# yanqinJiang/Animate3D

Hardware: AMD Instinct MI355X
Metric: UNet denoise-steps/sec, 4view×16frame×512² MV-VDM @1/2/4/8 GPU (higher is better)
Workload: dtype bf16; 1 GPU; BASELINE config 2: 4 views x 16 frames x 512^2 px (64x64 latent), CFG-doubled batch V=8 videos, one MVUNetMotionModel.forward per step, SD1.5 MV-VDM UNet 1.53 B params, seeded synthetic weights; parallelism=single GPU

## Files before the change

### animate3d_amd/csrc/gemm_common.h

```cpp
#pragma once
#include "common.h"

struct GemmParams {
  const uint16_t* X; int64_t ldx;
  const uint16_t* W; int64_t ldw;
  const float* bias;
  const uint16_t* rowbias; int64_t rb_div;
  const uint16_t* R; int64_t ldr;
  uint16_t* Y; int64_t ldy;
  int64_t M, N, K;
  float alpha, beta;
  int vec16;
  int out_f32;
  int B, H, Wd, Cin, Ho, Wo, stride, up, He, We;
  int64_t tiles_n, tiles_m;
  int ksplit, nk_item;
  float* ws; int64_t ws_bytes;
  const uint16_t* X2; int64_t ldx2; int64_t K1;
};

constexpr int EPI_LINEAR = 0, EPI_GEGLU = 1;

static inline int a3d_gemm_kernel_of(int flags) { return flags & A3D_GEMM_KERNEL_MASK; }
static inline int a3d_gemm_reserved_cus_of(int flags) { return flags & A3D_GEMM_RESERVED_CUS_MASK; }
// ... 101 lines not shown
      const int o = (i * 4) % BIAS_IMG_STRIDE;
      if ((o < BIAS_IMG_ROWBIAS && !bias) || (o >= BIAS_IMG_ROWBIAS && !rowbias)) bz[i] = 0u;
    }
    asm volatile("s_waitcnt lgkmcnt(0)" ::: "memory");
    tile_barrier();
  }
}

template <int NB> A3D_DEV void read_frags(const char* stage, uint32_t xrd, uint32_t wrd, uint32_t wrd_last, uint32_t ko, u32x4_t (&fx)[2],
                                          u32x4_t (&fw)[NB]) {
  const char* xs = stage + xrd;
  const char* ws = stage + wrd;
  const char* wl = stage + wrd_last;
#pragma unroll
  for (int tm = 0; tm < 2; ++tm) fx[tm] = *reinterpret_cast<const u32x4_t*>(xs + tm * 4096 + ko);
#pragma unroll
  for (int tn = 0; tn < NB - 1; ++tn) fw[tn] = *reinterpret_cast<const u32x4_t*>(ws + tn * 4096 + ko);
  fw[NB - 1] = *reinterpret_cast<const u32x4_t*>(wl + ko);
}

template <int EPI, int NB>
A3D_DEV void epilogue_rounded(const GemmParams& p, f32x16_t (&acc)[NB][2], float* const stg, const float* const bias_lds,
                              const uint16_t* const rowbias_lds, const int64_t m0, const int64_t n0, const int wm, const WaveCols<NB> wc,
                              const int lane) {
  const int wblk = wc.first, wblk_last = wc.last;
  auto pass_cols = [&](int ps) { return (2 * ps + 1 < NB) ? 64 : 32; };
  auto pass_col0 = [&](int ps) { return ((2 * ps + 1 < NB) ? wblk + 2 * ps : wblk_last) * 32; };
  const int l31 = lane & 31, g = lane >> 5;
  constexpr int NP = (NB + 1) / 2;
  constexpr int RS = (EPI == EPI_GEGLU) ? 64 : 128;
// ... 196 lines not shown
#pragma unroll
      for (int e = 0; e < 8; ++e) v[e] = epi_scale(v[e], p.alpha);
      const u32x4_t tr = rres[pi & 1][j];
#pragma unroll
      for (int e = 0; e < 4; ++e) { v[2 * e] = epi_axpy(v[2 * e], p.beta, lo16(tr[e])); v[2 * e + 1] = epi_axpy(v[2 * e + 1], p.beta, hi16(tr[e])); }
      u32x4_t o;
#pragma unroll
      for (int e = 0; e < 4; ++e) o[e] = pack16(v[2 * e], v[2 * e + 1]);
      *reinterpret_cast<u32x4_t*>(p.Y + m * p.ldy + n) = o;
    }
    wave_lds_fence();
  }
}


__attribute__((visibility("hidden"))) int A3D_FN(a3d_launch_gemm_pp)(int conv, int epi, int nb, hipStream_t stream, const GemmParams& p, int cus);
__attribute__((visibility("hidden"))) int A3D_FN(a3d_launch_gemm_ring)(int nb, hipStream_t stream, const GemmParams& p, int cus);
```

### animate3d_amd/csrc/gemm_conv.hip

```cpp
#include "gemm_common.h"

namespace {

constexpr int BM = 128, BN = 128;
template <int BKT> struct TileCfg {
  static constexpr int LROW = BKT + 8;
  static constexpr int TILE_ELEMS = 128 * LROW;
  static constexpr int STAGE_BYTES = 2 * 2 * TILE_ELEMS * 2;
  static constexpr int EPI_BYTES = 4 * 32 * 68 * 4;
  static constexpr int SMEM_BYTES = STAGE_BYTES > EPI_BYTES ? STAGE_BYTES : EPI_BYTES;
  static constexpr int CPR = BKT / 8;
  static constexpr int RPT = 256 / CPR;
  static constexpr int NPASS = 128 / RPT;
};



template <int CONV, int EPI, int BKT, bool RES>
__global__ __launch_bounds__(256, (BKT == 64 ? 2 : 3)) void gemm_kernel(const GemmParams p) {
  using TC = TileCfg<BKT>;
  constexpr int LROW = TC::LROW, TILE_ELEMS = TC::TILE_ELEMS, NPASS = TC::NPASS, RPT = TC::RPT, BK = BKT;
  extern __shared__ __attribute__((aligned(16))) uint16_t smem[];
  const int tid = threadIdx.x;
  const int lane = tid & 63, wid = tid >> 6;
// ... 277 lines not shown
            o[1] = pack16(w[2], w[3]);
            *reinterpret_cast<u32x2_t*>(yy + 4 * hh) = o;
          }
        }
      }
    }
  }
  if (tm == 0 && epf) prefetch_residual(1);
  }
}


constexpr int PBM = 256;
constexpr int NOT_ELIGIBLE = -1000;

inline bool gemm_flags_ok(int flags) {
  return !(flags & ~(A3D_GEMM_RESERVED_CUS_MASK | A3D_GEMM_KERNEL_MASK)) && a3d_gemm_kernel_of(flags) <= A3D_GEMM_RING;
}

inline int device_cus() {
  static int cus_of[64] = {0};
  const int dev = a3d_current_device();
  if (cus_of[dev] == 0) {
    int n = 0;
    if (hipDeviceGetAttribute(&n, hipDeviceAttributeMultiprocessorCount, dev) != hipSuccess) return 0;
    cus_of[dev] = n > 0 ? n : 256;
  }
  return cus_of[dev];
}

constexpr int PERSIST_MIN_FILL = 50;
struct PPPlan { int nb, S, cus; int64_t tiles_m, tiles_n; };
// ... 56 lines not shown
    if (p.N % (64 * nb) != 0) continue;
    const int64_t tiles = (p.M / 128) * (p.N / (64 * nb));
    const int64_t rounds = (tiles + out.cus - 1) / out.cus;
    const int64_t cost = rounds * (128 + 64 * nb);
    if (out.nb == 0 || cost < out.cost) { out.nb = nb; out.cost = cost; }
  }
  return out.nb != 0;
}

template <int CONV, int EPI>
int try_launch_persist(hipStream_t stream, GemmParams& p, int flags) {
  PPPlan pl;
  if (!plan_persist<CONV, EPI>(p, flags, p.ws != nullptr, pl)) return NOT_ELIGIBLE;
  p.tiles_m = pl.tiles_m; p.tiles_n = pl.tiles_n;
  p.ksplit = pl.S; p.nk_item = (int)(p.K / 64) / pl.S;
  return A3D_FN(a3d_launch_gemm_pp)(CONV, EPI, pl.nb, stream, p, pl.cus);
}


template <int CONV, int EPI, int BKT, bool RES>
int launch_res(hipStream_t stream, GemmParams& p, int64_t nblk) {
  using TC = TileCfg<BKT>;
  static uint64_t attr_done = 0;
  if (int rc = a3d_once_per_device(attr_done, [] {
        return (int)hipFuncSetAttribute(reinterpret_cast<const void*>(&gemm_kernel<CONV, EPI, BKT, RES>),
                                        hipFuncAttributeMaxDynamicSharedMemorySize, TC::SMEM_BYTES); })) return rc;
  gemm_kernel<CONV, EPI, BKT, RES><<<dim3((unsigned)nblk), dim3(256), TC::SMEM_BYTES, stream>>>(p);
  return a3d_launch_status();
}

template <int CONV, int EPI, int BKT>
int launch_bk(hipStream_t stream, GemmParams& p, int64_t nblk) {
  if constexpr (EPI == EPI_LINEAR) {
    if (p.R != nullptr) return launch_res<CONV, EPI, BKT, true>(stream, p, nblk);
  }
  return launch_res<CONV, EPI, BKT, false>(stream, p, nblk);
}

template <int CONV, int EPI = EPI_LINEAR>
int launch(hipStream_t stream, GemmParams& p, int flags) {
  if (!gemm_flags_ok(flags)) return A3D_EINVAL;
  if constexpr (CONV == 0 && EPI == EPI_LINEAR) {
    RingPlan rp;
    if (plan_ring(p, flags, rp)) {
      PPPlan pl;
      bool ring = true;
      if (a3d_gemm_kernel_of(flags) != A3D_GEMM_RING && plan_persist<CONV, EPI>(p, flags, p.ws != nullptr, pl)) {
        const int64_t tiles = pl.tiles_m * pl.tiles_n * pl.S;
        const int64_t pp_cost = ((tiles + rp.cus_plan - 1) / rp.cus_plan) * (256 + 64 * pl.nb) * RING_VS_PP_PCT;
        ring = pl.S == 1 && rp.cost * 100 < pp_cost;
      }
      if (ring) {
        p.tiles_m = p.M / 128; p.tiles_n = p.N / (64 * rp.nb);
        return A3D_FN(a3d_launch_gemm_ring)(rp.nb, stream, p, rp.cus);
      }
    }
// ... 4 lines not shown
  }
  p.tiles_m = (p.M + BM - 1) / BM;
  p.tiles_n = (p.N + BN - 1) / BN;
  const int64_t nblk = p.tiles_m * p.tiles_n;
  if (nblk <= 0 || nblk > 0x7fffffffLL) return A3D_EINVAL;
  const bool small = (CONV == 0 && p.K <= 640) || nblk < 768;
  if (small) return launch_bk<CONV, EPI, 32>(stream, p, nblk);
  return launch_bk<CONV, EPI, 64>(stream, p, nblk);
}

template <int CONV>
int64_t splitk_ws_bytes(const GemmParams& p, int flags) {
  PPPlan pl;
  GemmParams q = p;
  q.ws = nullptr; q.ws_bytes = 0;
  if (!gemm_flags_ok(flags)) return 0;
  if (!plan_persist<CONV, EPI_LINEAR>(q, flags, true, pl) || pl.S <= 1) return 0;
  return pl.tiles_m * pl.tiles_n * pl.S * pl.nb * 65536;
}

void attach_workspace(GemmParams& p, void* ws, int64_t ws_bytes) {
  if (ws && ws_bytes > 0 && a3d_aligned(16, ws)) { p.ws = (float*)ws; p.ws_bytes = ws_bytes; }
}

GemmParams dense_params(const void* X, int64_t ldx, const void* W, int64_t ldw, const float* bias, const void* rowbias, int64_t rb_div,
                        const void* R, int64_t ldr, void* Y, int64_t ldy, int64_t M, int64_t N, int64_t K, float alpha, float beta,
                        bool out_f32 = false) {
  GemmParams p{};
  p.X = (const uint16_t*)X; p.ldx = ldx; p.W = (const uint16_t*)W; p.ldw = ldw;
  p.bias = bias; p.rowbias = (const uint16_t*)rowbias; p.rb_div = rowbias ? rb_div : 1;
  p.R = (const uint16_t*)R; p.ldr = ldr; p.Y = (uint16_t*)Y; p.ldy = ldy;
// ... 30 lines not shown
  return gemm_entry(stream, X, ldx, W, ldw, bias, rowbias, rb_div, R, ldr, Y, ldy, M, N, K, alpha, beta, flags, nullptr, 0, nullptr);
}

extern "C" int A3D_FN(a3d_gemm_ws)(a3d_stream_t stream, const void* X, int64_t ldx, const void* W, int64_t ldw,
                                const float* bias, const void* rowbias, int64_t rb_div, const void* R, int64_t ldr,
                                void* Y, int64_t ldy, int64_t M, int64_t N, int64_t K, float alpha, float beta, int flags,
                                void* ws, int64_t ws_bytes, int64_t* ws_needed) {
  return gemm_entry(stream, X, ldx, W, ldw, bias, rowbias, rb_div, R, ldr, Y, ldy, M, N, K, alpha, beta, flags, ws, ws_bytes, ws_needed);
}

extern "C" int A3D_FN(a3d_gemm2)(a3d_stream_t stream, const void* X, int64_t ldx, const void* X2, int64_t ldx2, int64_t K1,
                              const void* W, int64_t ldw, const float* bias, void* Y, int64_t ldy, int64_t M, int64_t N, int64_t K, int flags) {
  GemmParams p = dense_params(X, ldx, W, ldw, bias, nullptr, 1, nullptr, 0, Y, ldy, M, N, K, 1.f, 0.f);
  p.X2 = (const uint16_t*)X2; p.ldx2 = ldx2; p.K1 = K1;
  if (!dense_args_ok(p, 16, 8, 8) || !X2 || K1 <= 0 || K1 >= K || K1 % 64 != 0 || ldx2 % 8 != 0 || !a3d_aligned(16, X2)) return A3D_EINVAL;
  if (!gemm_flags_ok(flags)) return A3D_EINVAL;
  if (ldx2 % 64 != 0 || (uint64_t)ldx2 * 16u >= (1ull << 31)) return A3D_EUNSUPPORTED;
  const int rc = try_launch_persist<0, EPI_LINEAR>((hipStream_t)stream, p, flags);
  return rc == NOT_ELIGIBLE ? A3D_EUNSUPPORTED : rc;
}

extern "C" int A3D_FN(a3d_gemm_f32out)(a3d_stream_t stream, const void* X, int64_t ldx, const void* W, int64_t ldw,
                                    const float* bias, float* Y, int64_t ldy, int64_t M, int64_t N, int64_t K, float alpha) {
  GemmParams p = dense_params(X, ldx, W, ldw, bias, nullptr, 1, nullptr, 0, Y, ldy, M, N, K, alpha, 0.f, true);
  if (!dense_args_ok(p, 16, 8, 4)) return A3D_EINVAL;
  return launch<0>((hipStream_t)stream, p, 0);
}

static int conv_entry(a3d_stream_t stream, const void* X, const void* Wp, const float* bias,
                      const void* rowbias, int64_t rb_div, const void* R, void* Y,
                      int B, int H, int W, int Cin, int Cout, int stride, int up2x, int flags,
// ... 42 lines not shown
```

### animate3d_amd/csrc/gemm_pp.hip

```cpp
#include "gemm_common.h"

namespace {

constexpr int PBM = 256;
template <int NB> struct PPCfg {
  static constexpr int BN = NB * 64;
  static constexpr int XBYTES = PBM * 128;
  static constexpr int WBYTES = BN * 128;
  static constexpr int EPI_BYTES = 8 * 32 * 68 * 4;
  static constexpr int STAGE = (XBYTES + WBYTES) > EPI_BYTES ? (XBYTES + WBYTES) : EPI_BYTES;
  static constexpr int BIAS_OFF = 2 * STAGE;
  static constexpr int SMEM = BIAS_OFF + 2 * BIAS_IMG_STRIDE;
};

constexpr int PP_GM = 8;
A3D_DEV void pp_tile_coords(int64_t t, int64_t tiles_m, int64_t tiles_n, int64_t& tile_m, int64_t& tile_n) {
  const int64_t gsz = PP_GM * tiles_n;
  const int64_t blk = t / gsz;
  const int64_t first = blk * PP_GM;
  const int64_t gm = tiles_m - first < PP_GM ? tiles_m - first : PP_GM;
  const int64_t within = t - blk * gsz;
  tile_n = within / gm;
  tile_m = first + (within - tile_n * gm);
}

template <int CONV, int EPI, int NB, bool RES, bool SPLIT = false, bool TWO = false>
__global__ __launch_bounds__(512, 1) void gemm_pp_kernel(const GemmParams p) {
  static_assert(!TWO || CONV == 0, "the two-source A operand is a dense-GEMM feature");
  using PC = PPCfg<NB>;
  constexpr int PH = 1, NPH = 4;
  constexpr int NP = 4 + NB;
  extern __shared__ __attribute__((aligned(16))) uint16_t smem[];
  char* const smem_b = reinterpret_cast<char*>(smem);
  const int tid = threadIdx.x, lane = tid & 63;
  const int wid = __builtin_amdgcn_readfirstlane(tid >> 6);
  const int wm = wid >> 1, wn = wid & 1;
  const int grp = wid >> 2;
  const int l31 = lane & 31, g = lane >> 5;
  const int lr = lane >> 3, pos = lane & 7;
  const uint32_t lds0 = lds_addr(smem);

  const int S = SPLIT ? p.ksplit : 1;
  const int64_t ntiles = p.tiles_m * p.tiles_n * S;
  const int64_t G = gridDim.x;
  int64_t t = xcd_remap(blockIdx.x, G);
  if (t >= ntiles) return;
// ... 13 lines not shown
  const int64_t cbias = CONV ? ((int64_t)p.Wd + 1) * p.Cin : 0;
  int64_t ld_m0 = 0, ld_n0 = 0;
  int ld_par = 0;
  int ik0 = 0, itap = 0, ikx = 0, iky = 0;
  uint64_t xck = 0;
  uint64_t zpage = 0;
  if constexpr (CONV != 0) {
    zpage = (uint64_t)(uintptr_t)g_zero_page;
    asm volatile("" : "+s"(zpage));
  }
  uint64_t xk = 0, wk = 0, rbk = 0;
  const uint32_t sx8 = (uint32_t)(p.ldx * 16), sw8 = (uint32_t)(p.ldw * 16);
  uint64_t xk2 = 0;
  const uint32_t vx0b = TWO ? (uint32_t)(lr * p.ldx2 * 2 + ((pos ^ (lr >> 1)) << 4)) : 0u;
  const uint32_t sx8b = TWO ? (uint32_t)(p.ldx2 * 16) : 0u;
  auto setup_tile = [&](int64_t tt) {
    int64_t tile_n, tile_m;
    const int64_t tile_id = SPLIT ? (int64_t)((uint32_t)tt / (uint32_t)S) : tt;
    const int64_t kofs = SPLIT ? (CONV ? ((int64_t)(tt - tile_id * S) * nk / 9) * 64 : (int64_t)(tt - tile_id * S) * nk * 64) : 0;
    pp_tile_coords(tile_id, p.tiles_m, p.tiles_n, tile_m, tile_n);
    ld_m0 = tile_m * PBM; ld_n0 = tile_n * PC::BN;
    ik0 = 0; itap = 0; ikx = 0; iky = 0;
    ld_par ^= 1;
    if constexpr (CONV != 0) xck = (uint64_t)(uintptr_t)p.X - (uint64_t)cbias * 2u + (uint64_t)kofs * 2u;
    if constexpr (CONV == 0) xk = (uint64_t)(uintptr_t)(p.X + (ld_m0 + wid * 32) * p.ldx + kofs);
    if constexpr (TWO) xk2 = (uint64_t)(uintptr_t)(p.X2 + (ld_m0 + wid * 32) * p.ldx2);
    wk = (uint64_t)(uintptr_t)(p.W + (ld_n0 + wid * (NB * 8)) * p.ldw + kofs);
    if (EPI == EPI_LINEAR && p.rowbias) rbk = (uint64_t)(uintptr_t)(p.rowbias + (ld_m0 / p.rb_div) * p.N + ld_n0);
    if constexpr (CONV != 0) {
      amask[0] = 0; amask[1] = 0;
#pragma unroll
      for (int i = 0; i < 4; ++i) {
        const int r = (wid * 4 + i) * 8 + lr;
        const int slot = pos ^ ((r >> 1) & 7);
        const uint32_t m = (uint32_t)ld_m0 + (uint32_t)r;
        const uint32_t hw = (uint32_t)(p.Ho * p.Wo);
        const int b = (int)(m / hw);
        const int rem = (int)(m - (uint32_t)b * hw);
        const int oy = (int)((uint32_t)rem / (uint32_t)p.Wo), ox = rem - oy * p.Wo;
        uint32_t mask = 0;
        if constexpr (CONV == 2) {
          const int sy0 = (oy - 1) >> 1, sx0 = (ox - 1) >> 1;
          aoff[i] = (uint32_t)(((((int64_t)b * p.H + sy0) * p.Wd + sx0) * p.Cin + cbias) * 2 + slot * 16);
#pragma unroll
// ... 25 lines not shown
    constexpr int A = decltype(a_c)::value, B = decltype(b_c)::value;
    if constexpr (A >= B) return;
    const uint32_t dst = lds0 + (uint32_t)buf * PC::STAGE;
    if constexpr (A == 0) {
      if (ik0 == 0) {
        const uint32_t bdst = lds0 + (uint32_t)PC::BIAS_OFF + (uint32_t)ld_par * BIAS_IMG_STRIDE;
        if (p.bias) {
          if (wid == 0) glds16_s((uint32_t)lane * 16u, p.bias + ld_n0, bdst);
          if (NB == 5 && wid == 1) { if (lane < 16) glds16_s((uint32_t)lane * 16u, p.bias + ld_n0 + BIAS_IMG_DMA / 4, bdst + (uint32_t)BIAS_IMG_DMA); }
        }
        if (EPI == EPI_LINEAR && p.rowbias && wid == 2) {
          if (lane < PC::BN / 8) glds16_s((uint32_t)lane * 16u, (const void*)(uintptr_t)rbk, bdst + (uint32_t)BIAS_IMG_ROWBIAS);
        }
      }
    }
    if constexpr (CONV != 0) {
      const int ky = iky, kx = ikx;
      const uint32_t rowb = (uint32_t)(p.Wd * p.Cin * 2), colb = (uint32_t)(p.Cin * 2);
      const uint32_t yE = (uint32_t)((ky + 1) >> 1) * rowb, yO = (uint32_t)(ky >> 1) * rowb;
      const uint32_t xE = (uint32_t)((kx + 1) >> 1) * colb, xO = (uint32_t)(kx >> 1) * colb;
#pragma unroll
      for (int i = 0; i < 4; ++i) {
        if (i < A || i >= B) continue;
        const uint32_t d = dst + (uint32_t)(wid * 4 + i) * 1024u;
        const uint32_t mk = amask[i >> 1];
        uint32_t vo = aoff[i];
        if constexpr (CONV == 2) vo += (((mk >> (18 + 2 * (i & 1))) & 1u) ? yE : yO) + (((mk >> (19 + 2 * (i & 1))) & 1u) ? xE : xO);
        const int bit = itap + 9 * (i & 1);
        if ((sok[i >> 1] >> bit) & 1u) {
          glds16_s(vo, (const void*)(uintptr_t)xck, d);
        } else {
// ... 2 lines not shown
        }
      }
    } else {
      const bool sec = TWO && ik0 >= (int)p.K1;
      const uint32_t vxs = sec ? vx0b : vx0, sxs = sec ? sx8b : sx8;
      const uint64_t xks = sec ? xk2 : xk;
#pragma unroll
      for (int i = 0; i < 4; ++i) {
        if (i < A || i >= B) continue;
        const int pc = wid * 4 + i;
        glds16_s(vxs ^ (uint32_t)((i & 1) << 6), (const void*)(uintptr_t)(xks + (uint64_t)(uint32_t)(i * sxs)), dst + (uint32_t)pc * 1024u);
      }
    }
#pragma unroll
    for (int i = 0; i < NB; ++i) {
      if (4 + i < A || 4 + i >= B) continue;
      const int pc = wid * NB + i;
      glds16_s(vw0 ^ (uint32_t)((pc & 1) << 6), (const void*)(uintptr_t)(wk + (uint64_t)(uint32_t)(i * sw8)), dst + (uint32_t)PC::XBYTES + (uint32_t)pc * 1024u);
    }
    if constexpr (B == NP) {
      if constexpr (CONV != 0) {
        const uint64_t cin2 = (uint64_t)(uint32_t)p.Cin * 2u;
        wk += cin2;
        ++itap;
        if (++ikx == 3) { ikx = 0; ++iky; }
        if (itap == 9) {
          itap = 0; iky = 0; wk -= 9u * cin2 - 128u;
          if constexpr (CONV == 1) xck -= (2u * (uint64_t)(uint32_t)p.Wd + 2u) * cin2;
          xck += 128u;
        } else if constexpr (CONV == 1) {
          xck += ikx == 0 ? ((uint64_t)(uint32_t)p.Wd - 2u) * cin2 : cin2;
        }
      } else {
        if (TWO && ik0 >= (int)p.K1) xk2 += 128; else xk += 128;
        wk += 128;
      }
      ik0 += 64;
    }
  };
  auto issue_phase = [&](int buf, auto ph_c, bool late) __attribute__((always_inline)) {
    constexpr int ph = decltype(ph_c)::value;
    using I0 = std::integral_constant<int, 0>;
    using I3 = std::integral_constant<int, 3>;
    using I5 = std::integral_constant<int, 5>;
    using I6 = std::integral_constant<int, 6>;
    using IN = std::integral_constant<int, NP>;
    if (!late) {
      if constexpr (ph == 0) issue_pieces(buf, I0{}, I3{});
      if constexpr (ph == 1) issue_pieces(buf, I3{}, I6{});
      if constexpr (ph == 2) issue_pieces(buf, I6{}, IN{});
    } else {
      if constexpr (ph == 1) issue_pieces(buf, I0{}, I5{});
      if constexpr (ph == 2) issue_pieces(buf, I5{}, IN{});
    }
  };

  f32x16_t acc[NB][2];
  u32x4_t fx[PH][2], fw[PH][NB];
  auto load_frags = [&](int buf, int ks0) __attribute__((always_inline)) {
#pragma unroll
    for (int s = 0; s < PH; ++s) read_frags<NB>(smem_b + buf * PC::STAGE, xrd, wrd, wrd_last, koff0 ^ (uint32_t)((ks0 + s) << 5), fx[s], fw[s]);
  };
  auto mfma_phase = [&]() __attribute__((always_inline)) {
#pragma unroll
    for (int s = 0; s < PH; ++s)
#pragma unroll
      for (int tn = 0; tn < NB; ++tn)
#pragma unroll
        for (int tm = 0; tm < 2; ++tm) acc[tn][tm] = mfma32(fw[s][tn], fx[s][tm], acc[tn][tm]);
  };

  zero_absent_bias_images<512>(smem_b + PC::BIAS_OFF, p.bias, EPI == EPI_LINEAR ? p.rowbias : nullptr, tid);
  setup_tile(t);
  issue_pieces(0, std::integral_constant<int, 0>{}, std::integral_constant<int, NP>{});
  asm volatile("s_waitcnt vmcnt(0)" ::: "memory");
  tile_barrier();
  int buf = 0;
  for (;;) {
    int64_t tile_n, tile_m;
    pp_tile_coords(SPLIT ? (int64_t)((uint32_t)t / (uint32_t)S) : t, p.tiles_m, p.tiles_n, tile_m, tile_n);
    const int64_t m0 = tile_m * PBM, n0 = tile_n * PC::BN;
    const int64_t tnext = t + G;
#pragma unroll
    for (int a = 0; a < NB; ++a)
#pragma unroll
      for (int b = 0; b < 2; ++b)
#pragma unroll
        for (int r = 0; r < 16; ++r) acc[a][b][r] = 0.f;
    const int cur_par = ld_par;
    if (grp) tile_barrier();
    for (int kt = 0; kt < nk; ++kt) {
      const bool last = kt + 1 >= nk;
      const bool more = !last || tnext < ntiles;
      const bool late = kt == 0;
      static_for<NPH>([&](auto ph_c) __attribute__((always_inline)) {
        constexpr int ph = decltype(ph_c)::value;
        load_frags(buf, ph * PH);
        if (more) {
          if constexpr (ph == 0 || ph == 1) {
            if (last && (late ? ph == 1 : ph == 0)) setup_tile(tnext);
          }
          issue_phase(buf ^ 1, ph_c, late);
          if constexpr (ph == NPH - 1) { if (grp) asm volatile("s_waitcnt vmcnt(0)" ::: "memory"); }
        }
        asm volatile("s_waitcnt lgkmcnt(0)" ::: "memory");
        tile_barrier();
        __builtin_amdgcn_s_setprio(1);
        mfma_phase();
        __builtin_amdgcn_s_setprio(0);
        __builtin_amdgcn_sched_barrier(0);
        if constexpr (ph == NPH - 1) { if (more && !grp) asm volatile("s_waitcnt vmcnt(0)" ::: "memory"); }
        tile_barrier();
      });
      buf ^= 1;
    }
    if (!grp) tile_barrier();

    if constexpr (SPLIT) {
      float* const wsi = p.ws + ((t * 8 + wid) * (NB * 8)) * 256 + lane * 4;
#pragma unroll
      for (int tn = 0; tn < NB; ++tn)
#pragma unroll
        for (int tm = 0; tm < 2; ++tm)
#pragma unroll
          for (int q = 0; q < 4; ++q)
            *reinterpret_cast<float4*>(wsi + ((tn * 2 + tm) * 4 + q) * 256) =
                float4{acc[tn][tm][4 * q], acc[tn][tm][4 * q + 1], acc[tn][tm][4 * q + 2], acc[tn][tm][4 * q + 3]};
    } else {
      float* const stg = reinterpret_cast<float*>(smem_b + (buf ^ 1) * PC::STAGE) + wid * (32 * 68);
      const float* const bias_lds = bias_image(smem_b + PC::BIAS_OFF, cur_par);
      const uint16_t* const rowbias_lds = rowbias_image(smem_b + PC::BIAS_OFF, cur_par);
      if constexpr (EPI == EPI_GEGLU || !RES) epilogue_rounded<EPI, NB>(p, acc, stg, bias_lds, rowbias_lds, m0, n0, wm, wc, lane);
      else epilogue_residual<NB>(p, acc, stg, bias_lds, rowbias_lds, m0, n0, wm, wc, lane);
    }
    if (tnext >= ntiles) break;
    t = tnext;
  }
}

template <int NB>
__global__ __launch_bounds__(512) void splitk_reduce_kernel(const GemmParams p) {
  using PC = PPCfg<NB>;
  const int tid = threadIdx.x, lane = tid & 63, wid = tid >> 6;
  const int wm = wid >> 1, wn = wid & 1, l31 = lane & 31, g = lane >> 5;
  const WaveCols<NB> wc(wn);
  const int S = p.ksplit;
  int64_t tile_n, tile_m;
  pp_tile_coords(blockIdx.x, p.tiles_m, p.tiles_n, tile_m, tile_n);
// ... 26 lines not shown
#pragma unroll
        for (int e = 0; e < 4; ++e) v[e] = epi_scale(v[e], p.alpha);
        if (p.R) {
          const u32x2_t tr = *reinterpret_cast<const u32x2_t*>(p.R + m * p.ldr + n);
          v[0] = epi_axpy(v[0], p.beta, lo16(tr[0])); v[1] = epi_axpy(v[1], p.beta, hi16(tr[0]));
          v[2] = epi_axpy(v[2], p.beta, lo16(tr[1])); v[3] = epi_axpy(v[3], p.beta, hi16(tr[1]));
        }
        u32x2_t o;
        o[0] = pack16(v[0], v[1]);
        o[1] = pack16(v[2], v[3]);
        *reinterpret_cast<u32x2_t*>(p.Y + m * p.ldy + n) = o;
      }
    }
}

template <int CONV, int EPI, int NB, bool RES, bool SPLIT = false, bool TWO = false>
int launch_pp(hipStream_t stream, const GemmParams& p, int cus) {
  using PC = PPCfg<NB>;
  static uint64_t attr_done = 0;
  if (int rc = a3d_once_per_device(attr_done, [] {
        return (int)hipFuncSetAttribute(reinterpret_cast<const void*>(&gemm_pp_kernel<CONV, EPI, NB, RES, SPLIT, TWO>),
                                        hipFuncAttributeMaxDynamicSharedMemorySize, PC::SMEM); })) return rc;
  const int64_t ntiles = p.tiles_m * p.tiles_n * (SPLIT ? p.ksplit : 1);
  const unsigned grid = (unsigned)(ntiles < cus ? ntiles : cus);
  gemm_pp_kernel<CONV, EPI, NB, RES, SPLIT, TWO><<<dim3(grid), dim3(512), PC::SMEM, stream>>>(p);
  if (int rc = a3d_launch_status()) return rc;
  if constexpr (SPLIT) {
    splitk_reduce_kernel<NB><<<dim3((unsigned)(p.tiles_m * p.tiles_n), NB), dim3(512), 0, stream>>>(p);
    return a3d_launch_status();
  }
  return 0;
}

template <int CONV>
int launch_pp_conv(int epi, int nb, hipStream_t stream, const GemmParams& p, int cus) {
  if (epi == EPI_GEGLU) {
    if constexpr (CONV == 0) { if (nb == 4) return launch_pp<0, EPI_GEGLU, 4, false>(stream, p, cus); }
    return A3D_EUNSUPPORTED;
  }
  if constexpr (CONV == 0) {
    if (p.X2 != nullptr) {
      if (p.R || p.ksplit > 1) return A3D_EUNSUPPORTED;
      if (nb == 5) return launch_pp<0, EPI_LINEAR, 5, false, false, true>(stream, p, cus);
      if (nb == 4) return launch_pp<0, EPI_LINEAR, 4, false, false, true>(stream, p, cus);
      return A3D_EUNSUPPORTED;
    }
  }
  if (p.ksplit > 1) {
    if (nb == 5) return launch_pp<CONV, EPI_LINEAR, 5, false, true>(stream, p, cus);
    if (nb == 4) return launch_pp<CONV, EPI_LINEAR, 4, false, true>(stream, p, cus);
    return A3D_EUNSUPPORTED;
  }
  if (nb == 5) return p.R ? launch_pp<CONV, EPI_LINEAR, 5, true>(stream, p, cus) : launch_pp<CONV, EPI_LINEAR, 5, false>(stream, p, cus);
  if (nb == 4) return p.R ? launch_pp<CONV, EPI_LINEAR, 4, true>(stream, p, cus) : launch_pp<CONV, EPI_LINEAR, 4, false>(stream, p, cus);
  return A3D_EUNSUPPORTED;
}

}

int A3D_FN(a3d_launch_gemm_pp)(int conv, int epi, int nb, hipStream_t stream, const GemmParams& p, int cus) {
  if (conv == 0) return launch_pp_conv<0>(epi, nb, stream, p, cus);
  if (conv == 1) return launch_pp_conv<1>(epi, nb, stream, p, cus);
  return launch_pp_conv<2>(epi, nb, stream, p, cus);
}
```

### animate3d_amd/hip_ops.py

```python
from __future__ import annotations

import ctypes
import os
from dataclasses import dataclass
from typing import Optional

import torch

_LIB_PATH = os.path.join(os.path.dirname(os.path.abspath(__file__)), "lib", "libanimate3d_hip.so")
_lib = None

c_i64, c_int, c_f32, c_f64, c_vp = ctypes.c_int64, ctypes.c_int, ctypes.c_float, ctypes.c_double, ctypes.c_void_p


class _RowMapC(ctypes.Structure):
    _fields_ = [("gdiv", c_i64), ("ga", c_i64), ("gb", c_i64), ("seg_len", c_i64), ("seg_stride", c_i64), ("ld", c_i64)]


@dataclass(frozen=True)
class RowMap:
    gdiv: int
    ga: int
    gb: int
    seg_len: int
# ... 273 lines not shown
        assert n % 32 == 0
        h, g = w[:n].reshape(n // 32, 32, *w.shape[1:]), w[n:].reshape(n // 32, 32, *w.shape[1:])
        return torch.stack([h, g], dim=1).reshape(w.shape).contiguous()

    def gemm_geglu(self, x, w_il, bias_il, *, tile128: bool = False):
        x, w_il = self._act(x, "geglu.x"), self._act(w_il, "geglu.w")
        M, K = x.shape
        N2 = w_il.shape[0]
        y = self.empty(M, N2 // 2)
        rc = self.lib.a3d_gemm_geglu_bf16(self._stream(), _p(x), x.stride(0), _p(w_il), w_il.stride(0), _p(bias_il), _p(y), y.stride(0), M, N2, K,
                                          self._gemm_flags(tile128))
        _check(rc, f"a3d_gemm_geglu_bf16 M={M} N2={N2} K={K}")
        return y

    def conv3x3(self, x, B: int, H: int, W: int, w, bias, *, stride: int = 1, up2x: bool = False, rowbias=None, rb_div: int = 1, residual=None,
                up_size=None, tile128: bool = False):
        x, w = self._act(x, "conv.x"), self._act(w, "conv.w")
        Cin = x.shape[1]
        Cout = w.shape[0]
        assert x.is_contiguous() and w.is_contiguous() and x.shape[0] == B * H * W and w.shape[1] == 9 * Cin
        He, We = (2 * H, 2 * W) if up2x else (H, W)
        up_code = 1 if up2x else 0
        if up_size is not None:
            if not up2x or up_size[0] not in (2 * H, 2 * H - 1) or up_size[1] not in (2 * W, 2 * W - 1):
                raise ValueError(f"forced upsample size {tuple(up_size)} is not reachable from {(H, W)} (2x or 2x - 1 per axis)")
            He, We = int(up_size[0]), int(up_size[1])
            up_code |= (2 if He == 2 * H - 1 else 0) | (4 if We == 2 * W - 1 else 0)
        Ho, Wo = (He - 1) // stride + 1, (We - 1) // stride + 1
        y = self.empty(B * Ho * Wo, Cout)
        if residual is not None:
            assert residual.is_contiguous() and residual.shape == y.shape
        if rowbias is not None:
            assert rowbias.is_contiguous() and rowbias.shape[1] == Cout
        flags = self._gemm_flags(tile128)
        args = (self._stream(), _p(x), _p(w), _p(bias), _p(rowbias), rb_div, _p(residual), _p(y), B, H, W, Cin, Cout, stride, up_code, flags)
        if self.split_k and not tile128 and B * Ho * Wo <= 32768:
            key = ("conv", B, H, W, Cin, Cout, stride, up_code, rb_div if rowbias is not None else 0, flags)
            need = self._ws_plan.get(key)
            if need is None:
                q = c_i64(0)
                _check(self.lib.a3d_conv3x3_ws_bf16(*args, None, 0, ctypes.byref(q)), f"a3d_conv3x3_ws_bf16 (query) B={B} H={H} W={W} Cin={Cin} Cout={Cout}")
                need = self._ws_plan[key] = int(q.value)
            if need > 0:
                ws = self._workspace(need)
                _check(self.lib.a3d_conv3x3_ws_bf16(*args, _p(ws), need, None), f"a3d_conv3x3_ws_bf16 B={B} H={H} W={W} Cin={Cin} Cout={Cout}")
                return y, Ho, Wo
        rc = self.lib.a3d_conv3x3_bf16(*args)
        _check(rc, f"a3d_conv3x3_bf16 B={B} H={H} W={W} Cin={Cin} Cout={Cout} stride={stride} up={up2x}")
        return y, Ho, Wo
# ... 410 lines not shown
```

### include/animate3d_hip.h

```cpp
#ifndef ANIMATE3D_HIP_H
#define ANIMATE3D_HIP_H

#include <stdint.h>

#ifdef __cplusplus
extern "C" {
#endif

typedef void* a3d_stream_t;

enum {
  A3D_OK = 0,
  A3D_EINVAL = -1,
  A3D_EUNSUPPORTED = -2
};

enum { A3D_F32 = 0, A3D_BF16 = 1, A3D_F16 = 2 };

const char* a3d_version(void);

typedef struct a3d_rowmap {
  int64_t gdiv, ga, gb;
  int64_t seg_len, seg_stride;
  int64_t ld;
} a3d_rowmap;

#define A3D_GEMM_RESERVED_CUS_MASK 0xff
#define A3D_GEMM_KERNEL_MASK 0x300
#define A3D_GEMM_TILE128 0x100
#define A3D_GEMM_RING 0x200
int a3d_gemm_bf16(a3d_stream_t stream, const void* X, int64_t ldx, const void* W, int64_t ldw,
                  const float* bias, const void* rowbias, int64_t rb_div, const void* R, int64_t ldr,
                  void* Y, int64_t ldy, int64_t M, int64_t N, int64_t K, float alpha, float beta, int flags);

int a3d_gemm_ws_bf16(a3d_stream_t stream, const void* X, int64_t ldx, const void* W, int64_t ldw,
                     const float* bias, const void* rowbias, int64_t rb_div, const void* R, int64_t ldr,
                     void* Y, int64_t ldy, int64_t M, int64_t N, int64_t K, float alpha, float beta, int flags,
                     void* ws, int64_t ws_bytes, int64_t* ws_needed);

int a3d_gemm2_bf16(a3d_stream_t stream, const void* X, int64_t ldx, const void* X2, int64_t ldx2, int64_t K1,
                   const void* W, int64_t ldw, const float* bias, void* Y, int64_t ldy, int64_t M, int64_t N, int64_t K, int flags);

int a3d_gemm_f32out_bf16(a3d_stream_t stream, const void* X, int64_t ldx, const void* W, int64_t ldw,
                         const float* bias, float* Y, int64_t ldy, int64_t M, int64_t N, int64_t K, float alpha);

// ... 291 lines not shown
```

Measured before the change: 2.404 denoise-steps/s.

## Stage conv input row windows in LDS once per K-chunk for stride-1 3x3 convs

Adds a window-staged variant of the persistent implicit-GEMM conv kernel. For stride-1 convs with 64- or 32-wide images and 320-column tiles, it loads the needed input rows into an LDS window once per 64-channel chunk and reads all nine taps from it, instead of re-gathering the A tile from global memory for every tap. This cuts global and L2 traffic for the A operand and frees the X staging area, at the cost of complex row-slot double-buffering and epilogue buffers placed in the window region. A per-tap flag keeps the old path available.

```diff
diff --git a/animate3d_amd/csrc/gemm_common.h b/animate3d_amd/csrc/gemm_common.h
--- a/animate3d_amd/csrc/gemm_common.h
+++ b/animate3d_amd/csrc/gemm_common.h
@@ -139,6 +139,17 @@
   const char* wl = stage + wrd_last;
 #pragma unroll
   for (int tm = 0; tm < 2; ++tm) fx[tm] = *reinterpret_cast<const u32x4_t*>(xs + tm * 4096 + ko);
+#pragma unroll
+  for (int tn = 0; tn < NB - 1; ++tn) fw[tn] = *reinterpret_cast<const u32x4_t*>(ws + tn * 4096 + ko);
+  fw[NB - 1] = *reinterpret_cast<const u32x4_t*>(wl + ko);
+}
+
+template <int NB> A3D_DEV void read_frags_w(const char* stage, const char* xs0, const char* xs1, uint32_t wrd, uint32_t wrd_last, uint32_t ko,
+                                            u32x4_t (&fx)[2], u32x4_t (&fw)[NB]) {
+  const char* ws = stage + wrd;
+  const char* wl = stage + wrd_last;
+  fx[0] = *reinterpret_cast<const u32x4_t*>(xs0);
+  fx[1] = *reinterpret_cast<const u32x4_t*>(xs1);
 #pragma unroll
   for (int tn = 0; tn < NB - 1; ++tn) fw[tn] = *reinterpret_cast<const u32x4_t*>(ws + tn * 4096 + ko);
   fw[NB - 1] = *reinterpret_cast<const u32x4_t*>(wl + ko);
@@ -365,5 +376,5 @@
 }
 
 
-__attribute__((visibility("hidden"))) int A3D_FN(a3d_launch_gemm_pp)(int conv, int epi, int nb, hipStream_t stream, const GemmParams& p, int cus);
+__attribute__((visibility("hidden"))) int A3D_FN(a3d_launch_gemm_pp)(int conv, int epi, int nb, bool win, hipStream_t stream, const GemmParams& p, int cus);
 __attribute__((visibility("hidden"))) int A3D_FN(a3d_launch_gemm_ring)(int nb, hipStream_t stream, const GemmParams& p, int cus);
diff --git a/animate3d_amd/csrc/gemm_conv.hip b/animate3d_amd/csrc/gemm_conv.hip
--- a/animate3d_amd/csrc/gemm_conv.hip
+++ b/animate3d_amd/csrc/gemm_conv.hip
@@ -315,8 +315,8 @@
 constexpr int PBM = 256;
 constexpr int NOT_ELIGIBLE = -1000;
 
-inline bool gemm_flags_ok(int flags) {
-  return !(flags & ~(A3D_GEMM_RESERVED_CUS_MASK | A3D_GEMM_KERNEL_MASK)) && a3d_gemm_kernel_of(flags) <= A3D_GEMM_RING;
+inline bool gemm_flags_ok(int flags, bool conv) {
+  return !(flags & ~(A3D_GEMM_RESERVED_CUS_MASK | A3D_GEMM_KERNEL_MASK | (conv ? A3D_CONV_PER_TAP : 0))) && a3d_gemm_kernel_of(flags) <= A3D_GEMM_RING;
 }
 
 inline int device_cus() {
@@ -403,7 +403,9 @@
   if (!plan_persist<CONV, EPI>(p, flags, p.ws != nullptr, pl)) return NOT_ELIGIBLE;
   p.tiles_m = pl.tiles_m; p.tiles_n = pl.tiles_n;
   p.ksplit = pl.S; p.nk_item = (int)(p.K / 64) / pl.S;
-  return A3D_FN(a3d_launch_gemm_pp)(CONV, EPI, pl.nb, stream, p, pl.cus);
+  const bool win = CONV == 1 && p.stride == 1 && !(flags & A3D_CONV_PER_TAP) && pl.nb == 5 && pl.S == 1 && (p.Wd == 64 || p.Wd == 32) &&
+                   ((int64_t)p.H * p.Wd) % PBM == 0;
+  return A3D_FN(a3d_launch_gemm_pp)(CONV, EPI, pl.nb, win, stream, p, pl.cus);
 }
 
 
@@ -428,7 +430,7 @@
 
 template <int CONV, int EPI = EPI_LINEAR>
 int launch(hipStream_t stream, GemmParams& p, int flags) {
-  if (!gemm_flags_ok(flags)) return A3D_EINVAL;
+  if (!gemm_flags_ok(flags, CONV != 0)) return A3D_EINVAL;
   if constexpr (CONV == 0 && EPI == EPI_LINEAR) {
     RingPlan rp;
     if (plan_ring(p, flags, rp)) {
@@ -463,7 +465,7 @@
   PPPlan pl;
   GemmParams q = p;
   q.ws = nullptr; q.ws_bytes = 0;
-  if (!gemm_flags_ok(flags)) return 0;
+  if (!gemm_flags_ok(flags, CONV != 0)) return 0;
   if (!plan_persist<CONV, EPI_LINEAR>(q, flags, true, pl) || pl.S <= 1) return 0;
   return pl.tiles_m * pl.tiles_n * pl.S * pl.nb * 65536;
 }
@@ -524,7 +526,7 @@
   GemmParams p = dense_params(X, ldx, W, ldw, bias, nullptr, 1, nullptr, 0, Y, ldy, M, N, K, 1.f, 0.f);
   p.X2 = (const uint16_t*)X2; p.ldx2 = ldx2; p.K1 = K1;
   if (!dense_args_ok(p, 16, 8, 8) || !X2 || K1 <= 0 || K1 >= K || K1 % 64 != 0 || ldx2 % 8 != 0 || !a3d_aligned(16, X2)) return A3D_EINVAL;
-  if (!gemm_flags_ok(flags)) return A3D_EINVAL;
+  if (!gemm_flags_ok(flags, false)) return A3D_EINVAL;
   if (ldx2 % 64 != 0 || (uint64_t)ldx2 * 16u >= (1ull << 31)) return A3D_EUNSUPPORTED;
   const int rc = try_launch_persist<0, EPI_LINEAR>((hipStream_t)stream, p, flags);
   return rc == NOT_ELIGIBLE ? A3D_EUNSUPPORTED : rc;
diff --git a/animate3d_amd/csrc/gemm_pp.hip b/animate3d_amd/csrc/gemm_pp.hip
--- a/animate3d_amd/csrc/gemm_pp.hip
+++ b/animate3d_amd/csrc/gemm_pp.hip
@@ -3,15 +3,30 @@
 namespace {
 
 constexpr int PBM = 256;
-template <int NB> struct PPCfg {
+template <int NB, bool WIN = false> struct PPCfg {
   static constexpr int BN = NB * 64;
-  static constexpr int XBYTES = PBM * 128;
+  static constexpr int XBYTES = WIN ? 0 : PBM * 128;
   static constexpr int WBYTES = BN * 128;
-  static constexpr int EPI_BYTES = 8 * 32 * 68 * 4;
-  static constexpr int STAGE = (XBYTES + WBYTES) > EPI_BYTES ? (XBYTES + WBYTES) : EPI_BYTES;
-  static constexpr int BIAS_OFF = 2 * STAGE;
+  static constexpr int EPI_WAVE = 32 * 68 * 4;
+  static constexpr int EPI_BYTES = 8 * EPI_WAVE;
+  static constexpr int STAGE = WIN ? WBYTES : ((XBYTES + WBYTES) > EPI_BYTES ? (XBYTES + WBYTES) : EPI_BYTES);
+  static constexpr int WIN_OFF = 2 * STAGE;
+  static constexpr int WIN_BYTES = WIN ? 16 * 34 * 128 : 0;
+  static constexpr int BIAS_OFF = WIN_OFF + WIN_BYTES;
   static constexpr int SMEM = BIAS_OFF + 2 * BIAS_IMG_STRIDE;
+  static_assert(!WIN || (4 * EPI_WAVE <= WBYTES && 4 * EPI_WAVE <= WIN_BYTES / 2), "window-staged conv: the epilogue buffers do not fit");
+  static_assert(SMEM <= 160 * 1024, "LDS plan exceeds the CU's 160 KB");
 };
+
+constexpr uint64_t win_jobs(int a0, int a1, int a2, int a3, int a4, int a5, int a6, int a7, int a8) {
+  const int a[9] = {a0, a1, a2, a3, a4, a5, a6, a7, a8};
+  uint64_t v = 0;
+  for (int i = 0; i < 9; ++i) v |= (uint64_t)(a[i] & 15) << (4 * i);
+  return v;
+}
+constexpr uint64_t WIN_JOBS_64 = win_jobs(4, 5, 2, 0, 3, 15, 1, 15, 15);
+constexpr uint64_t WIN_JOBS_32E = win_jobs(8, 2, 4, 0, 6, 15, 15, 15, 15);
+constexpr uint64_t WIN_JOBS_32O = win_jobs(9, 3, 5, 15, 7, 15, 1, 15, 15);
 
 constexpr int PP_GM = 8;
 A3D_DEV void pp_tile_coords(int64_t t, int64_t tiles_m, int64_t tiles_n, int64_t& tile_m, int64_t& tile_n) {
@@ -24,12 +39,14 @@
   tile_m = first + (within - tile_n * gm);
 }
 
-template <int CONV, int EPI, int NB, bool RES, bool SPLIT = false, bool TWO = false>
+template <int CONV, int EPI, int NB, bool RES, bool SPLIT = false, bool TWO = false, bool WIN = false>
 __global__ __launch_bounds__(512, 1) void gemm_pp_kernel(const GemmParams p) {
   static_assert(!TWO || CONV == 0, "the two-source A operand is a dense-GEMM feature");
-  using PC = PPCfg<NB>;
+  static_assert(!WIN || (CONV == 1 && !SPLIT && NB == 5), "the window-staged A operand serves unsplit stride-1 convs with 320-column tiles");
+  using PC = PPCfg<NB, WIN>;
   constexpr int PH = 1, NPH = 4;
-  constexpr int NP = 4 + NB;
+  constexpr int XP = WIN ? 0 : 4;
+  constexpr int NP = XP + NB;
   extern __shared__ __attribute__((aligned(16))) uint16_t smem[];
   char* const smem_b = reinterpret_cast<char*>(smem);
   const int tid = threadIdx.x, lane = tid & 63;
@@ -73,6 +90,42 @@
   uint64_t xk2 = 0;
   const uint32_t vx0b = TWO ? (uint32_t)(lr * p.ldx2 * 2 + ((pos ^ (lr >> 1)) << 4)) : 0u;
   const uint32_t sx8b = TWO ? (uint32_t)(p.ldx2 * 16) : 0u;
+  const int wR = WIN ? PBM / p.Wd : 1;
+  const uint32_t wSL = WIN ? (uint32_t)PC::WIN_BYTES / (2u * (uint32_t)wR) : 0u;
+  const int wcol = WIN ? (wid & ((p.Wd >> 3) - 1)) : 0;
+  const int wcls = WIN && p.Wd == 32 ? wid >> 2 : 0;
+  const uint64_t wtab = !WIN ? 0 : p.Wd == 64 ? WIN_JOBS_64 : wcls ? WIN_JOBS_32O : WIN_JOBS_32E;
+  const uint32_t vwin = WIN ? (uint32_t)((lr + wcol * 8) * p.Cin * 2 + ((pos ^ (lr >> 1) ^ ((wcol & 1) << 2)) << 4)) : 0u;
+  const uint32_t wdst0 = lds0 + (uint32_t)PC::WIN_OFF + (uint32_t)(1 + wcol * 8) * 128u;
+  const uint32_t xwin = (uint32_t)PC::WIN_OFF + (uint32_t)(((wm * 64) & (p.Wd - 1)) + l31) * 128u;
+  const int wj0 = WIN ? (wm * 64) / p.Wd : 0, wj1 = WIN ? (wm * 64 + 32) / p.Wd : 0;
+  const uint32_t wx1 = WIN && p.Wd == 64 ? 32u * 128u : 0u;
+  uint64_t wb_cur = 0, wb_nxt = 0;
+  int ty_cur = 0, ty_nxt = 0;
+  int nxt_ok = 0;
+  int cpar = 0;
+  int ct = 0, cdy = 0, cdx = 0;
+  uint32_t xa[2] = {0u, 0u}, kofw = 0u;
+  auto win_tile = [&](int64_t tt, uint64_t& wb, int& ty) {
+    int64_t tile_n, tile_m;
+    pp_tile_coords(tt, p.tiles_m, p.tiles_n, tile_m, tile_n);
+    const uint32_t m = (uint32_t)tile_m * (uint32_t)PBM;
+    wb = (uint64_t)(uintptr_t)p.X + (uint64_t)m * (uint64_t)(uint32_t)(p.Cin * 2);
+    ty = (int)((m / (uint32_t)p.Wd) % (uint32_t)p.H);
+  };
+  auto issue_win_row = [&](int j, int par, uint64_t wb, int ty) __attribute__((always_inline)) {
+    const int yy = ty + j - 1;
+    const bool in = yy >= 0 && yy < p.H;
+    const int slot = j + ((par && j >= 2 && j < wR) ? wR : 0);
+    const uint64_t src = in ? wb + (uint64_t)((int64_t)(j - 1) * (int64_t)(p.Wd * p.Cin * 2)) : zpage;
+    glds16_s(in ? vwin : 0u, (const void*)(uintptr_t)src, wdst0 + (uint32_t)slot * wSL);
+  };
+  auto issue_win_job = [&]() __attribute__((always_inline)) {
+    const int j = (int)((wtab >> (4 * ct)) & 15u);
+    if (j == 15) return;
+    if (j >= wR) issue_win_row(j, cpar, wb_cur, ty_cur);
+    else if (nxt_ok) issue_win_row(j, cpar ^ 1, wb_nxt, ty_nxt);
+  };
   auto setup_tile = [&](int64_t tt) {
     int64_t tile_n, tile_m;
     const int64_t tile_id = SPLIT ? (int64_t)((uint32_t)tt / (uint32_t)S) : tt;
@@ -81,12 +134,12 @@
     ld_m0 = tile_m * PBM; ld_n0 = tile_n * PC::BN;
     ik0 = 0; itap = 0; ikx = 0; iky = 0;
     ld_par ^= 1;
-    if constexpr (CONV != 0) xck = (uint64_t)(uintptr_t)p.X - (uint64_t)cbias * 2u + (uint64_t)kofs * 2u;
+    if constexpr (CONV != 0 && !WIN) xck = (uint64_t)(uintptr_t)p.X - (uint64_t)cbias * 2u + (uint64_t)kofs * 2u;
     if constexpr (CONV == 0) xk = (uint64_t)(uintptr_t)(p.X + (ld_m0 + wid * 32) * p.ldx + kofs);
     if constexpr (TWO) xk2 = (uint64_t)(uintptr_t)(p.X2 + (ld_m0 + wid * 32) * p.ldx2);
     wk = (uint64_t)(uintptr_t)(p.W + (ld_n0 + wid * (NB * 8)) * p.ldw + kofs);
     if (EPI == EPI_LINEAR && p.rowbias) rbk = (uint64_t)(uintptr_t)(p.rowbias + (ld_m0 / p.rb_div) * p.N + ld_n0);
-    if constexpr (CONV != 0) {
+    if constexpr (CONV != 0 && !WIN) {
       amask[0] = 0; amask[1] = 0;
 #pragma unroll
       for (int i = 0; i < 4; ++i) {
@@ -142,7 +195,8 @@
         }
       }
     }
-    if constexpr (CONV != 0) {
+    if constexpr (WIN) {
+    } else if constexpr (CONV != 0) {
       const int ky = iky, kx = ikx;
       const uint32_t rowb = (uint32_t)(p.Wd * p.Cin * 2), colb = (uint32_t)(p.Cin * 2);
       const uint32_t yE = (uint32_t)((ky + 1) >> 1) * rowb, yO = (uint32_t)(ky >> 1) * rowb;
@@ -175,7 +229,7 @@
     }
 #pragma unroll
     for (int i = 0; i < NB; ++i) {
-      if (4 + i < A || 4 + i >= B) continue;
+      if (XP + i < A || XP + i >= B) continue;
       const int pc = wid * NB + i;
       glds16_s(vw0 ^ (uint32_t)((pc & 1) << 6), (const void*)(uintptr_t)(wk + (uint64_t)(uint32_t)(i * sw8)), dst + (uint32_t)PC::XBYTES + (uint32_t)pc * 1024u);
     }
@@ -187,9 +241,9 @@
         if (++ikx == 3) { ikx = 0; ++iky; }
         if (itap == 9) {
           itap = 0; iky = 0; wk -= 9u * cin2 - 128u;
-          if constexpr (CONV == 1) xck -= (2u * (uint64_t)(uint32_t)p.Wd + 2u) * cin2;
+          if constexpr (CONV == 1 && !WIN) xck -= (2u * (uint64_t)(uint32_t)p.Wd + 2u) * cin2;
           xck += 128u;
-        } else if constexpr (CONV == 1) {
+        } else if constexpr (CONV == 1 && !WIN) {
           xck += ikx == 0 ? ((uint64_t)(uint32_t)p.Wd - 2u) * cin2 : cin2;
         }
       } else {
@@ -202,15 +256,17 @@
   auto issue_phase = [&](int buf, auto ph_c, bool late) __attribute__((always_inline)) {
     constexpr int ph = decltype(ph_c)::value;
     using I0 = std::integral_constant<int, 0>;
-    using I3 = std::integral_constant<int, 3>;
-    using I5 = std::integral_constant<int, 5>;
-    using I6 = std::integral_constant<int, 6>;
+    using I3 = std::integral_constant<int, WIN ? 1 : 3>;
+    using I5 = std::integral_constant<int, WIN ? 2 : 5>;
+    using I6 = std::integral_constant<int, WIN ? 3 : 6>;
     using IN = std::integral_constant<int, NP>;
     if (!late) {
+      if constexpr (WIN && ph == 0) issue_win_job();
       if constexpr (ph == 0) issue_pieces(buf, I0{}, I3{});
       if constexpr (ph == 1) issue_pieces(buf, I3{}, I6{});
       if constexpr (ph == 2) issue_pieces(buf, I6{}, IN{});
     } else {
+      if constexpr (WIN && ph == 1) issue_win_job();
       if constexpr (ph == 1) issue_pieces(buf, I0{}, I5{});
       if constexpr (ph == 2) issue_pieces(buf, I5{}, IN{});
     }
@@ -220,7 +276,15 @@
   u32x4_t fx[PH][2], fw[PH][NB];
   auto load_frags = [&](int buf, int ks0) __attribute__((always_inline)) {
 #pragma unroll
-    for (int s = 0; s < PH; ++s) read_frags<NB>(smem_b + buf * PC::STAGE, xrd, wrd, wrd_last, koff0 ^ (uint32_t)((ks0 + s) << 5), fx[s], fw[s]);
+    for (int s = 0; s < PH; ++s) {
+      if constexpr (WIN) {
+        const uint32_t kw = kofw ^ (uint32_t)((ks0 + s) << 5);
+        read_frags_w<NB>(smem_b + buf * PC::STAGE, smem_b + xa[0] + kw, smem_b + xa[1] + kw, wrd, wrd_last, koff0 ^ (uint32_t)((ks0 + s) << 5),
+                         fx[s], fw[s]);
+      } else {
+        read_frags<NB>(smem_b + buf * PC::STAGE, xrd, wrd, wrd_last, koff0 ^ (uint32_t)((ks0 + s) << 5), fx[s], fw[s]);
+      }
+    }
   };
   auto mfma_phase = [&]() __attribute__((always_inline)) {
 #pragma unroll
@@ -233,7 +297,17 @@
 
   zero_absent_bias_images<512>(smem_b + PC::BIAS_OFF, p.bias, EPI == EPI_LINEAR ? p.rowbias : nullptr, tid);
   setup_tile(t);
+  if constexpr (WIN) {
+    if (tid < 2 * wR * 16) {
+      const int slot = tid >> 4, side = (tid >> 3) & 1, c = tid & 7;
+      *reinterpret_cast<u32x4_t*>(smem_b + PC::WIN_OFF + (uint32_t)slot * wSL + (side ? (uint32_t)(p.Wd + 1) * 128u : 0u) + c * 16) = u32x4_t{0u, 0u, 0u, 0u};
+    }
+    win_tile(t, wb_cur, ty_cur);
+#pragma unroll
+    for (int q = 0; q < 4; ++q) issue_win_row(p.Wd == 64 ? q : wcls + 2 * q, 0, wb_cur, ty_cur);
+  }
   issue_pieces(0, std::integral_constant<int, 0>{}, std::integral_constant<int, NP>{});
+  if constexpr (WIN) asm volatile("s_waitcnt lgkmcnt(0)" ::: "memory");
   asm volatile("s_waitcnt vmcnt(0)" ::: "memory");
   tile_barrier();
   int buf = 0;
@@ -254,6 +328,18 @@
       const bool last = kt + 1 >= nk;
       const bool more = !last || tnext < ntiles;
       const bool late = kt == 0;
+      if constexpr (WIN) {
+        if (ct == 0) {
+          if (kt + 9 < nk) { wb_nxt = wb_cur + 128u; ty_nxt = ty_cur; nxt_ok = 1; }
+          else if (tnext < ntiles) { win_tile(tnext, wb_nxt, ty_nxt); nxt_ok = 1; }
+          else nxt_ok = 0;
+        }
+        const int ja = wj0 + cdy, jb = wj1 + cdy;
+        const uint32_t sa = (uint32_t)(ja + ((cpar && ja >= 2 && ja < wR) ? wR : 0)) * wSL + (uint32_t)cdx * 128u;
+        const uint32_t sb = (uint32_t)(jb + ((cpar && jb >= 2 && jb < wR) ? wR : 0)) * wSL + (uint32_t)cdx * 128u + wx1;
+        xa[0] = xwin + sa; xa[1] = xwin + sb;
+        kofw = (uint32_t)((g ^ (((l31 + cdx + 15) >> 1) & 7)) << 4);
+      }
       static_for<NPH>([&](auto ph_c) __attribute__((always_inline)) {
         constexpr int ph = decltype(ph_c)::value;
         load_frags(buf, ph * PH);
@@ -274,6 +360,11 @@
         tile_barrier();
       });
       buf ^= 1;
+      if constexpr (WIN) {
+        ++ct;
+        if (++cdx == 3) { cdx = 0; ++cdy; }
+        if (ct == 9) { ct = 0; cdy = 0; cpar ^= 1; wb_cur = wb_nxt; ty_cur = ty_nxt; }
+      }
     }
     if (!grp) tile_barrier();
 
@@ -288,11 +379,19 @@
             *reinterpret_cast<float4*>(wsi + ((tn * 2 + tm) * 4 + q) * 256) =
                 float4{acc[tn][tm][4 * q], acc[tn][tm][4 * q + 1], acc[tn][tm][4 * q + 2], acc[tn][tm][4 * q + 3]};
     } else {
-      float* const stg = reinterpret_cast<float*>(smem_b + (buf ^ 1) * PC::STAGE) + wid * (32 * 68);
+      float* stg = reinterpret_cast<float*>(smem_b + (buf ^ 1) * PC::STAGE) + wid * (32 * 68);
+      const uint32_t wfree = (uint32_t)PC::WIN_OFF + (uint32_t)(cpar ? 2 : wR) * wSL + (uint32_t)((wid & 3) * PC::EPI_WAVE);
+      if constexpr (WIN) { if (wid >= 4) stg = reinterpret_cast<float*>(smem_b + wfree); }
       const float* const bias_lds = bias_image(smem_b + PC::BIAS_OFF, cur_par);
       const uint16_t* const rowbias_lds = rowbias_image(smem_b + PC::BIAS_OFF, cur_par);
       if constexpr (EPI == EPI_GEGLU || !RES) epilogue_rounded<EPI, NB>(p, acc, stg, bias_lds, rowbias_lds, m0, n0, wm, wc, lane);
       else epilogue_residual<NB>(p, acc, stg, bias_lds, rowbias_lds, m0, n0, wm, wc, lane);
+      if constexpr (WIN) {
+        if (wid >= 4 && lane < PC::EPI_WAVE / (int)wSL * 16) {
+          const int slot = lane >> 4, side = (lane >> 3) & 1, c = lane & 7;
+          *reinterpret_cast<u32x4_t*>(smem_b + wfree + (uint32_t)slot * wSL + (side ? (uint32_t)(p.Wd + 1) * 128u : 0u) + c * 16) = u32x4_t{0u, 0u, 0u, 0u};
+        }
+      }
     }
     if (tnext >= ntiles) break;
     t = tnext;
@@ -349,16 +448,16 @@
     }
 }
 
-template <int CONV, int EPI, int NB, bool RES, bool SPLIT = false, bool TWO = false>
+template <int CONV, int EPI, int NB, bool RES, bool SPLIT = false, bool TWO = false, bool WIN = false>
 int launch_pp(hipStream_t stream, const GemmParams& p, int cus) {
-  using PC = PPCfg<NB>;
+  using PC = PPCfg<NB, WIN>;
   static uint64_t attr_done = 0;
   if (int rc = a3d_once_per_device(attr_done, [] {
-        return (int)hipFuncSetAttribute(reinterpret_cast<const void*>(&gemm_pp_kernel<CONV, EPI, NB, RES, SPLIT, TWO>),
+        return (int)hipFuncSetAttribute(reinterpret_cast<const void*>(&gemm_pp_kernel<CONV, EPI, NB, RES, SPLIT, TWO, WIN>),
                                         hipFuncAttributeMaxDynamicSharedMemorySize, PC::SMEM); })) return rc;
   const int64_t ntiles = p.tiles_m * p.tiles_n * (SPLIT ? p.ksplit : 1);
   const unsigned grid = (unsigned)(ntiles < cus ? ntiles : cus);
-  gemm_pp_kernel<CONV, EPI, NB, RES, SPLIT, TWO><<<dim3(grid), dim3(512), PC::SMEM, stream>>>(p);
+  gemm_pp_kernel<CONV, EPI, NB, RES, SPLIT, TWO, WIN><<<dim3(grid), dim3(512), PC::SMEM, stream>>>(p);
   if (int rc = a3d_launch_status()) return rc;
   if constexpr (SPLIT) {
     splitk_reduce_kernel<NB><<<dim3((unsigned)(p.tiles_m * p.tiles_n), NB), dim3(512), 0, stream>>>(p);
@@ -368,7 +467,15 @@
 }
 
 template <int CONV>
-int launch_pp_conv(int epi, int nb, hipStream_t stream, const GemmParams& p, int cus) {
+int launch_pp_conv(int epi, int nb, bool win, hipStream_t stream, const GemmParams& p, int cus) {
+  if (win) {
+    if constexpr (CONV == 1) {
+      if (epi == EPI_LINEAR && nb == 5 && p.ksplit <= 1 && p.stride == 1)
+        return p.R ? launch_pp<1, EPI_LINEAR, 5, true, false, false, true>(stream, p, cus)
+                   : launch_pp<1, EPI_LINEAR, 5, false, false, false, true>(stream, p, cus);
+    }
+    return A3D_EUNSUPPORTED;
+  }
   if (epi == EPI_GEGLU) {
     if constexpr (CONV == 0) { if (nb == 4) return launch_pp<0, EPI_GEGLU, 4, false>(stream, p, cus); }
     return A3D_EUNSUPPORTED;
@@ -393,8 +500,8 @@
 
 }
 
-int A3D_FN(a3d_launch_gemm_pp)(int conv, int epi, int nb, hipStream_t stream, const GemmParams& p, int cus) {
-  if (conv == 0) return launch_pp_conv<0>(epi, nb, stream, p, cus);
-  if (conv == 1) return launch_pp_conv<1>(epi, nb, stream, p, cus);
-  return launch_pp_conv<2>(epi, nb, stream, p, cus);
-}
+int A3D_FN(a3d_launch_gemm_pp)(int conv, int epi, int nb, bool win, hipStream_t stream, const GemmParams& p, int cus) {
+  if (conv == 0) return launch_pp_conv<0>(epi, nb, win, stream, p, cus);
+  if (conv == 1) return launch_pp_conv<1>(epi, nb, win, stream, p, cus);
+  return launch_pp_conv<2>(epi, nb, win, stream, p, cus);
+}
diff --git a/animate3d_amd/hip_ops.py b/animate3d_amd/hip_ops.py
--- a/animate3d_amd/hip_ops.py
+++ b/animate3d_amd/hip_ops.py
@@ -311,7 +311,7 @@
         return y
 
     def conv3x3(self, x, B: int, H: int, W: int, w, bias, *, stride: int = 1, up2x: bool = False, rowbias=None, rb_div: int = 1, residual=None,
-                up_size=None, tile128: bool = False):
+                up_size=None, tile128: bool = False, per_tap: bool = False):
         x, w = self._act(x, "conv.x"), self._act(w, "conv.w")
         Cin = x.shape[1]
         Cout = w.shape[0]
@@ -329,7 +329,7 @@
             assert residual.is_contiguous() and residual.shape == y.shape
         if rowbias is not None:
             assert rowbias.is_contiguous() and rowbias.shape[1] == Cout
-        flags = self._gemm_flags(tile128)
+        flags = self._gemm_flags(tile128) | (0x800 if per_tap else 0)
         args = (self._stream(), _p(x), _p(w), _p(bias), _p(rowbias), rb_div, _p(residual), _p(y), B, H, W, Cin, Cout, stride, up_code, flags)
         if self.split_k and not tile128 and B * Ho * Wo <= 32768:
             key = ("conv", B, H, W, Cin, Cout, stride, up_code, rb_div if rowbias is not None else 0, flags)
diff --git a/include/animate3d_hip.h b/include/animate3d_hip.h
--- a/include/animate3d_hip.h
+++ b/include/animate3d_hip.h
@@ -29,6 +29,7 @@
 #define A3D_GEMM_KERNEL_MASK 0x300
 #define A3D_GEMM_TILE128 0x100
 #define A3D_GEMM_RING 0x200
+#define A3D_CONV_PER_TAP 0x800
 int a3d_gemm_bf16(a3d_stream_t stream, const void* X, int64_t ldx, const void* W, int64_t ldw,
                   const float* bias, const void* rowbias, int64_t rb_div, const void* R, int64_t ldr,
                   void* Y, int64_t ldy, int64_t M, int64_t N, int64_t K, float alpha, float beta, int flags);
```

Measured after the change: 2.413 denoise-steps/s (median of 6 runs). No clear change (+0.4%).
